# yl-jiang/YOLOSeries

Measured on AMD Instinct MI355X. Metric: images/sec (640x640) YOLOv5s train-step, higher is better.
Workload: dtype bf16; 1 GPU; YOLOv5s bf16 train step (fwd+loss+bwd+clip+SGD+EMA), batch 64/GPU x 640x640 synthetic COCO-80, random-init (BASELINE.json configs[1]); global_batch=64, parallelism=dp1

## Files before the change

yoloseries_amd/csrc/arena.hip:

```cpp
#include "common.h"
#include <stdarg.h>

namespace {
constexpr int TH = 256;
inline int grid_for(long n) {
    long g = (n + TH - 1) / TH;
    if (g > 4096) g = 4096;
    if (g < 1) g = 1;
    return (int)g;
}

__global__ void pack_bf16_kernel(const float* __restrict__ src, const int32_t* __restrict__ idx, long n, uint16_t* __restrict__ dst)
{
    const long n8 = ((reinterpret_cast<uintptr_t>(dst) | reinterpret_cast<uintptr_t>(idx)) & 15) ? 0 : n >> 3;
    for (long c = (long)blockIdx.x * blockDim.x + threadIdx.x; c < n8; c += (long)gridDim.x * blockDim.x) {
        const int4 j0 = *reinterpret_cast<const int4*>(idx + c * 8), j1 = *reinterpret_cast<const int4*>(idx + c * 8 + 4);
        const int j[8] = {j0.x, j0.y, j0.z, j0.w, j1.x, j1.y, j1.z, j1.w};
        float f[8];
#pragma unroll
        for (int e = 0; e < 8; ++e) f[e] = j[e] >= 0 ? src[j[e]] : 0.f;
        uint4 v;
        v.x = (uint32_t)f2bf(f[0]) | ((uint32_t)f2bf(f[1]) << 16);
        v.y = (uint32_t)f2bf(f[2]) | ((uint32_t)f2bf(f[3]) << 16);
        v.z = (uint32_t)f2bf(f[4]) | ((uint32_t)f2bf(f[5]) << 16);
        v.w = (uint32_t)f2bf(f[6]) | ((uint32_t)f2bf(f[7]) << 16);
        *reinterpret_cast<uint4*>(dst + c * 8) = v;
    }
    for (long i = n8 * 8 + (long)blockIdx.x * blockDim.x + threadIdx.x; i < n; i += (long)gridDim.x * blockDim.x) {
        int32_t j = idx[i];
        dst[i] = j >= 0 ? f2bf(src[j]) : (uint16_t)0;
    }
}
__global__ void gather_f32_kernel(const float* __restrict__ src, const int32_t* __restrict__ idx, long n, float* __restrict__ dst)
{
    const long n4 = ((reinterpret_cast<uintptr_t>(dst) | reinterpret_cast<uintptr_t>(idx)) & 15) ? 0 : n >> 2;
    for (long c = (long)blockIdx.x * blockDim.x + threadIdx.x; c < n4; c += (long)gridDim.x * blockDim.x) {
        const int4 j = *reinterpret_cast<const int4*>(idx + c * 4);
        float4 v;
        v.x = j.x >= 0 ? src[j.x] : 0.f; v.y = j.y >= 0 ? src[j.y] : 0.f; v.z = j.z >= 0 ? src[j.z] : 0.f; v.w = j.w >= 0 ? src[j.w] : 0.f;
        *reinterpret_cast<float4*>(dst + c * 4) = v;
    }
    for (long i = n4 * 4 + (long)blockIdx.x * blockDim.x + threadIdx.x; i < n; i += (long)gridDim.x * blockDim.x) {
        int32_t j = idx[i];
        dst[i] = j >= 0 ? src[j] : 0.f;
    }
}
__global__ void sgd_kernel(float* __restrict__ p, const float* __restrict__ g, float* __restrict__ buf,
                           const uint8_t* __restrict__ group, long n, const float* __restrict__ lr,
                           const float* __restrict__ wd, float momentum, int nesterov, int first,
                           const float* __restrict__ grad_scale)
{
    const float gs = grad_scale ? *grad_scale : 1.f;
    for (long i = (long)blockIdx.x * blockDim.x + threadIdx.x; i < n; i += (long)gridDim.x * blockDim.x) {
        int gi = group ? group[i] : 0;
        float pv = p[i];
        float gv = g[i] * gs + wd[gi] * pv;
        float b = first ? gv : momentum * buf[i] + gv;
        buf[i] = b;
        float upd = nesterov ? gv + momentum * b : b;
        p[i] = pv - lr[gi] * upd;
    }
}
__global__ void sgd_dev_kernel(float* __restrict__ p, const float* __restrict__ g, float* __restrict__ buf,
                               const uint8_t* __restrict__ group, long n, const float* __restrict__ scal, int nesterov,
                               const float* __restrict__ grad_scale)
{
    const float gs = grad_scale ? *grad_scale : 1.f;
    const float lr[3] = {scal[0], scal[1], scal[2]}, wd[3] = {scal[3], scal[4], scal[5]};
    const float momentum = scal[6];
    const bool first = scal[7] != 0.f;
    for (long i = (long)blockIdx.x * blockDim.x + threadIdx.x; i < n; i += (long)gridDim.x * blockDim.x) {
        int gi = group ? group[i] : 0;
        gi = gi > 2 ? 2 : gi;
        float pv = p[i];
        float gv = g[i] * gs + (gi == 0 ? wd[0] : (gi == 1 ? wd[1] : wd[2])) * pv;
        float b = first ? gv : momentum * buf[i] + gv;
        buf[i] = b;
        float upd = nesterov ? gv + momentum * b : b;
        p[i] = pv - (gi == 0 ? lr[0] : (gi == 1 ? lr[1] : lr[2])) * upd;
    }
}
__global__ void ema_dev_kernel(float* __restrict__ e, const float* __restrict__ p, long n, const float* __restrict__ decay_dev)
{
    const float decay = *decay_dev;
    for (long i = (long)blockIdx.x * blockDim.x + threadIdx.x; i < n; i += (long)gridDim.x * blockDim.x)
        e[i] = decay * e[i] + (1.f - decay) * p[i];
}
__global__ void ema_advance_kernel(long long* __restrict__ counter, float* __restrict__ decay, double ratio, double tau)
{
    if (threadIdx.x == 0 && blockIdx.x == 0) {
        const long long n = counter[0] + 1;
        counter[0] = n;
        decay[0] = (float)(ratio * (1.0 - exp(-(double)n / tau)));
    }
}
__global__ __launch_bounds__(TH) void sumsq_part_kernel(const float* __restrict__ x, long n, float* __restrict__ part)
{
    __shared__ double sw[TH / 64];
    double s = 0.0;
    for (long i = (long)blockIdx.x * blockDim.x + threadIdx.x; i < n; i += (long)gridDim.x * blockDim.x) {
        float v = x[i];
        s += (double)v * (double)v;
    }
    s = wave_sum_d(s);
    if ((threadIdx.x & 63) == 0) sw[threadIdx.x >> 6] = s;
    __syncthreads();
    if (threadIdx.x == 0) {
        double tsum = 0.0;
        for (int w = 0; w < TH / 64; ++w) tsum += sw[w];
        part[blockIdx.x] = (float)tsum;
    }
}
__global__ __launch_bounds__(256) void sum_final_kernel(const float* __restrict__ part, int nb, float* out)
{
    __shared__ double sw[4];
    double s = 0.0;
    for (int i = threadIdx.x; i < nb; i += 256) s += (double)part[i];
    s = wave_sum_d(s);
    if ((threadIdx.x & 63) == 0) sw[threadIdx.x >> 6] = s;
    __syncthreads();
    if (threadIdx.x == 0) *out = (float)(sw[0] + sw[1] + sw[2] + sw[3]);
}
__global__ void clip_scale_kernel(const float* sumsq, float max_norm, float* out)
{
    if (threadIdx.x == 0 && blockIdx.x == 0) {
        float c = max_norm / (sqrtf(*sumsq) + 1e-6f);
        *out = c < 1.f ? c : 1.f;
    }
}
__global__ void ema_kernel(float* __restrict__ e, const float* __restrict__ p, long n, float decay)
{
    for (long i = (long)blockIdx.x * blockDim.x + threadIdx.x; i < n; i += (long)gridDim.x * blockDim.x)
        e[i] = decay * e[i] + (1.f - decay) * p[i];
}
}

static thread_local char g_err[512] = "";
void yh_set_error(const char* fmt, ...) {
    va_list ap;
    va_start(ap, fmt);
    vsnprintf(g_err, sizeof(g_err), fmt, ap);
    va_end(ap);
}
extern "C" const char* yh_last_error(void) { return g_err; }
extern "C" int yh_version(void) { return 100; }
extern "C" int yh_device_cus(void) {
    int dev = 0;
    hipDeviceProp_t prop;
    if (hipGetDevice(&dev) != hipSuccess) return -1;
    if (hipGetDeviceProperties(&prop, dev) != hipSuccess) return -1;
    return prop.multiProcessorCount;
}

extern "C" int yh_pack_bf16(const float* src, const int32_t* idx, int64_t n, yh_bf16* dst, yh_stream stream)
{
    YH_CHECK_ARG(src && idx && dst && n >= 0, "yh_pack_bf16: bad args");
    if (n == 0) return YH_OK;
    hipLaunchKernelGGL(pack_bf16_kernel, dim3(grid_for(n)), dim3(TH), 0, (hipStream_t)stream, src, idx, (long)n, dst);
    YH_CHECK_LAUNCH("yh_pack_bf16");
    return YH_OK;
}
extern "C" int yh_gather_f32(const float* src, const int32_t* idx, int64_t n, float* dst, yh_stream stream)
{
    YH_CHECK_ARG(src && idx && dst && n >= 0, "yh_gather_f32: bad args");
    if (n == 0) return YH_OK;
    hipLaunchKernelGGL(gather_f32_kernel, dim3(grid_for(n)), dim3(TH), 0, (hipStream_t)stream, src, idx, (long)n, dst);
    YH_CHECK_LAUNCH("yh_gather_f32");
    return YH_OK;
}
extern "C" int yh_sgd_step(float* p, const float* g, float* buf, const uint8_t* group, int64_t n,
                           const float* lr, const float* wd, int ngroups, float momentum, int nesterov,
                           int first_step, const float* grad_scale, yh_stream stream)
{
    YH_CHECK_ARG(p && g && buf && lr && wd && n >= 0 && ngroups >= 1 && ngroups <= 256, "yh_sgd_step: bad args");
    if (n == 0) return YH_OK;
    hipLaunchKernelGGL(sgd_kernel, dim3(grid_for(n)), dim3(TH), 0, (hipStream_t)stream,
                       p, g, buf, group, (long)n, lr, wd, momentum, nesterov, first_step, grad_scale);
    YH_CHECK_LAUNCH("yh_sgd_step");
    return YH_OK;
}
extern "C" int yh_sgd_step_dev(float* p, const float* g, float* buf, const uint8_t* group, int64_t n,
                               const float* scal, int nesterov, const float* grad_scale, yh_stream stream)
{
    YH_CHECK_ARG(p && g && buf && scal && n >= 0, "yh_sgd_step_dev: bad args");
    if (n == 0) return YH_OK;
    hipLaunchKernelGGL(sgd_dev_kernel, dim3(grid_for(n)), dim3(TH), 0, (hipStream_t)stream, p, g, buf, group, (long)n, scal, nesterov, grad_scale);
    YH_CHECK_LAUNCH("yh_sgd_step_dev");
    return YH_OK;
}
extern "C" int yh_ema_update_dev(float* ema, const float* p, int64_t n, const float* decay_dev, yh_stream stream)
{
    YH_CHECK_ARG(ema && p && decay_dev && n >= 0, "yh_ema_update_dev: bad args");
    if (n == 0) return YH_OK;
    hipLaunchKernelGGL(ema_dev_kernel, dim3(grid_for(n)), dim3(TH), 0, (hipStream_t)stream, ema, p, (long)n, decay_dev);
    YH_CHECK_LAUNCH("yh_ema_update_dev");
    return YH_OK;
}
extern "C" int yh_ema_advance(int64_t* counter, float* decay, double ratio, double tau, yh_stream stream)
{
    YH_CHECK_ARG(counter && decay && tau > 0.0, "yh_ema_advance: bad args");
    hipLaunchKernelGGL(ema_advance_kernel, dim3(1), dim3(64), 0, (hipStream_t)stream, (long long*)counter, decay, ratio, tau);
    YH_CHECK_LAUNCH("yh_ema_advance");
    return YH_OK;
}
extern "C" int yh_sumsq(const float* x, int64_t n, float* part, float* out, yh_stream stream)
{
    YH_CHECK_ARG(x && part && out && n > 0, "yh_sumsq: bad args (part needs 4096 floats)");
    int nb = grid_for(n);
    hipLaunchKernelGGL(sumsq_part_kernel, dim3(nb), dim3(TH), 0, (hipStream_t)stream, x, (long)n, part);
    hipLaunchKernelGGL(sum_final_kernel, dim3(1), dim3(256), 0, (hipStream_t)stream, part, nb, out);
    YH_CHECK_LAUNCH("yh_sumsq");
    return YH_OK;
}
extern "C" int yh_ema_update(float* ema, const float* p, int64_t n, float decay, yh_stream stream)
{
    YH_CHECK_ARG(ema && p && n >= 0, "yh_ema_update: bad args");
    if (n == 0) return YH_OK;
    hipLaunchKernelGGL(ema_kernel, dim3(grid_for(n)), dim3(TH), 0, (hipStream_t)stream, ema, p, (long)n, decay);
    YH_CHECK_LAUNCH("yh_ema_update");
    return YH_OK;
}

extern "C" int yh_clip_scale(const float* sumsq, float max_norm, float* out, yh_stream stream)
{
    YH_CHECK_ARG(sumsq && out && max_norm > 0.f, "yh_clip_scale: bad args");
    hipLaunchKernelGGL(clip_scale_kernel, dim3(1), dim3(64), 0, (hipStream_t)stream, sumsq, max_norm, out);
    YH_CHECK_LAUNCH("yh_clip_scale");
    return YH_OK;
}
```

Before: 5404 images/sec.

## Stage contiguous source window in LDS for bf16 pack gather

Reworks the fp32-to-bf16 gather/pack kernel so each block handles a fixed segment of indices. It computes the min/max source index of the segment, loads that source range into shared memory with vectorised float4 reads, then gathers from LDS instead of doing scattered global loads. If the range does not fit the window it falls back to direct global gathers. This adds extra barriers and atomics per segment and changes the grid sizing to one block per segment.

```diff
diff --git a/yoloseries_amd/csrc/arena.hip b/yoloseries_amd/csrc/arena.hip
--- a/yoloseries_amd/csrc/arena.hip
+++ b/yoloseries_amd/csrc/arena.hip
@@ -10,21 +10,97 @@
     return (int)g;
 }
 
-__global__ void pack_bf16_kernel(const float* __restrict__ src, const int32_t* __restrict__ idx, long n, uint16_t* __restrict__ dst)
-{
+#ifndef YH_PK_SEG
+#define YH_PK_SEG 4096
+#endif
+#ifndef YH_PK_WIN
+#define YH_PK_WIN 9216
+#endif
+constexpr int PK_SEG = YH_PK_SEG;
+constexpr int PK_WIN = YH_PK_WIN;
+constexpr int PK_CH = PK_SEG / 8 / TH;
+constexpr int PK_QT = PK_WIN / 4 / TH;
+static_assert(PK_SEG % (8 * TH) == 0 && PK_CH >= 1 && PK_WIN % (4 * TH) == 0 && PK_WIN * 4 <= 64 * 1024, "pack_bf16: segment / window sizes");
+
+__device__ __forceinline__ uint4 pack_bf16x8(const float* f)
+{
+    uint4 v;
+    v.x = (uint32_t)f2bf(f[0]) | ((uint32_t)f2bf(f[1]) << 16);
+    v.y = (uint32_t)f2bf(f[2]) | ((uint32_t)f2bf(f[3]) << 16);
+    v.z = (uint32_t)f2bf(f[4]) | ((uint32_t)f2bf(f[5]) << 16);
+    v.w = (uint32_t)f2bf(f[6]) | ((uint32_t)f2bf(f[7]) << 16);
+    return v;
+}
+
+__global__ __launch_bounds__(TH) void pack_bf16_kernel(const float* __restrict__ src, const int32_t* __restrict__ idx, long n, uint16_t* __restrict__ dst)
+{
+    __shared__ float win[PK_WIN];
+    __shared__ int s_lo, s_hi;
     const long n8 = ((reinterpret_cast<uintptr_t>(dst) | reinterpret_cast<uintptr_t>(idx)) & 15) ? 0 : n >> 3;
-    for (long c = (long)blockIdx.x * blockDim.x + threadIdx.x; c < n8; c += (long)gridDim.x * blockDim.x) {
-        const int4 j0 = *reinterpret_cast<const int4*>(idx + c * 8), j1 = *reinterpret_cast<const int4*>(idx + c * 8 + 4);
-        const int j[8] = {j0.x, j0.y, j0.z, j0.w, j1.x, j1.y, j1.z, j1.w};
-        float f[8];
-#pragma unroll
-        for (int e = 0; e < 8; ++e) f[e] = j[e] >= 0 ? src[j[e]] : 0.f;
-        uint4 v;
-        v.x = (uint32_t)f2bf(f[0]) | ((uint32_t)f2bf(f[1]) << 16);
-        v.y = (uint32_t)f2bf(f[2]) | ((uint32_t)f2bf(f[3]) << 16);
-        v.z = (uint32_t)f2bf(f[4]) | ((uint32_t)f2bf(f[5]) << 16);
-        v.w = (uint32_t)f2bf(f[6]) | ((uint32_t)f2bf(f[7]) << 16);
-        *reinterpret_cast<uint4*>(dst + c * 8) = v;
+    const long nseg = (n8 * 8 + PK_SEG - 1) / PK_SEG;
+    const int t = threadIdx.x;
+    for (long sg = blockIdx.x; sg < nseg; sg += gridDim.x) {
+        if (t == 0) { s_lo = 0x7fffffff; s_hi = -1; }
+        __syncthreads();
+        int j[PK_CH][8];
+        int lo = 0x7fffffff, hi = -1;
+#pragma unroll
+        for (int k = 0; k < PK_CH; ++k) {
+            const long c = sg * (PK_SEG / 8) + k * TH + t;
+            const bool ok = c < n8;
+            const long cc = ok ? c : n8 - 1;
+            const int4 j0 = *reinterpret_cast<const int4*>(idx + cc * 8), j1 = *reinterpret_cast<const int4*>(idx + cc * 8 + 4);
+            const int jj[8] = {j0.x, j0.y, j0.z, j0.w, j1.x, j1.y, j1.z, j1.w};
+#pragma unroll
+            for (int e = 0; e < 8; ++e) {
+                j[k][e] = ok ? jj[e] : -1;
+                lo = j[k][e] >= 0 && j[k][e] < lo ? j[k][e] : lo;
+                hi = j[k][e] > hi ? j[k][e] : hi;
+            }
+        }
+        if (hi >= 0) { atomicMin(&s_lo, lo); atomicMax(&s_hi, hi); }
+        __syncthreads();
+        const long wlo = s_lo, whi = s_hi;
+        const long a0 = wlo - (long)(((reinterpret_cast<uintptr_t>(src) >> 2) + (uintptr_t)wlo) & 3);
+        const bool none = whi < 0;
+        const bool fits = none || whi - a0 < PK_WIN;
+        if (fits && !none) {
+            const int nq = (int)((whi - a0) / 4) + 1;
+            if (nq > 2) {
+                float4 v[PK_QT];
+#pragma unroll
+                for (int i = 0; i < PK_QT; ++i) {
+                    const int q = 1 + t + i * TH;
+                    const int qc = q < nq - 2 ? q : nq - 2;
+                    v[i] = *reinterpret_cast<const float4*>(src + a0 + 4L * qc);
+                }
+#pragma unroll
+                for (int i = 0; i < PK_QT; ++i) {
+                    const int q = 1 + t + i * TH;
+                    if (q <= nq - 2) *reinterpret_cast<float4*>(win + 4 * q) = v[i];
+                }
+            }
+            if (t < 8) {
+                const int q = t < 4 ? 0 : nq - 1;
+                const long p = a0 + 4L * q + (t & 3);
+                win[4 * q + (t & 3)] = (p >= wlo && p <= whi) ? src[p] : 0.f;
+            }
+        }
+        __syncthreads();
+#pragma unroll
+        for (int k = 0; k < PK_CH; ++k) {
+            const long c = sg * (PK_SEG / 8) + k * TH + t;
+            float f[8];
+            if (fits) {
+#pragma unroll
+                for (int e = 0; e < 8; ++e) f[e] = j[k][e] >= 0 ? win[j[k][e] - a0] : 0.f;
+            } else {
+#pragma unroll
+                for (int e = 0; e < 8; ++e) f[e] = j[k][e] >= 0 ? src[j[k][e]] : 0.f;
+            }
+            if (c < n8) *reinterpret_cast<uint4*>(dst + c * 8) = pack_bf16x8(f);
+        }
+        __syncthreads();
     }
     for (long i = n8 * 8 + (long)blockIdx.x * blockDim.x + threadIdx.x; i < n; i += (long)gridDim.x * blockDim.x) {
         int32_t j = idx[i];
@@ -156,7 +232,10 @@
 {
     YH_CHECK_ARG(src && idx && dst && n >= 0, "yh_pack_bf16: bad args");
     if (n == 0) return YH_OK;
-    hipLaunchKernelGGL(pack_bf16_kernel, dim3(grid_for(n)), dim3(TH), 0, (hipStream_t)stream, src, idx, (long)n, dst);
+    const bool vec = (((uintptr_t)dst | (uintptr_t)idx) & 15) == 0 && n >= 8;
+    const long nseg = ((n >> 3) * 8 + PK_SEG - 1) / PK_SEG;
+    const int grid = vec ? (int)(nseg < 4096 ? nseg : 4096) : grid_for(n);
+    hipLaunchKernelGGL(pack_bf16_kernel, dim3(grid), dim3(TH), 0, (hipStream_t)stream, src, idx, (long)n, dst);
     YH_CHECK_LAUNCH("yh_pack_bf16");
     return YH_OK;
 }
```

Measured after the change: 5382 images/sec. About the same (-0.4%).
